# sadit/Jchemo.jl

Hardware: AMD Instinct MI355X
Metric: latent-variables/sec (plskern n=1e6 p=500 q=10 nlv=25) (higher is better)
Workload: dtype f64

## Files before the change

### jchemo.jl_amd/csrc/fit.hip

```cpp
#include <stdlib.h>
#include <time.h>

#include <algorithm>
#include <condition_variable>
#include <mutex>
#include <thread>

#include "jch_internal.h"

__global__ __launch_bounds__(256) void k_fill_const(double *__restrict__ v, int m, double c)
{
    const int j = blockIdx.x * 256 + threadIdx.x;
    if (j < m) v[j] = c;
}

__global__ __launch_bounds__(256) void k_nan_zero_weight_rows(double *__restrict__ T, int64_t n, int nlv, const double *__restrict__ d)
{
    const int64_t i = (int64_t)blockIdx.x * 256 + threadIdx.x;
    if (i < n && d[i] == 0.0)
        for (int a = 0; a < nlv; ++a) T[(size_t)i + (size_t)a * (size_t)n] = __builtin_nan("");
}

__global__ __launch_bounds__(256) void k_widen_bf16(const unsigned short *__restrict__ src, int64_t ld, int64_t n, int64_t cols, double *__restrict__ dst)
{
// ... 151 lines not shown
    const bool host = d.loc == JCH_LOC_HOST;
    const bool inplace = d.inplace != 0;
    ctx->ev_used = 0;
    ctx->prof = jch_profile{};
    jch_coll_reset(ctx);
    ctx->sweep_seq = 0;
    ctx->sweep_alt = jch_knob("JCH_SWEEP_ALT", 0);
    ctx->sweep_fused_reduce = jch_knob("JCH_SWEEP_FUSED_REDUCE", 0) == 1;
    ctx->sweep_resident_mb = jch_knob("JCH_SWEEP_RESIDENT_MB", -1);
    ctx->sweep_tstage = jch_knob("JCH_SWEEP_TSTAGE", -1);
    const bool host_timing = jch_knob_set("JCH_HOST_TIMING");
    auto now_ms = [] { timespec ts; clock_gettime(CLOCK_MONOTONIC, &ts); return ts.tv_sec * 1e3 + ts.tv_nsec * 1e-6; };
    const double tl0 = now_ms();
    double tl_h2d = tl0, tl_enq = tl0, tl_sync = tl0;

    const xcopy_key xkey{io.X, (int64_t)n, (int64_t)io.ldx, p, host ? 1 : 0};
    const bool reuse_x = (d.reserved & JCH_REUSE_XCOPY) && allow_raw && ctx->xcopy_valid && ctx->xcopy == xkey && d.dtype == JCH_F64 &&
                         q + 1 <= 12 && ldr <= 512 && !jch_knob_set("JCH_NO_REUSE_XCOPY");
    if (!reuse_x) ctx->xcopy_valid = false;
    double *Xc = (double *)io.X, *Yc = (double *)io.Y;
    const double *wdev = io.weights;
    int64_t ldxc = io.ldx, ldyc = io.ldy;
    if (host) {
        JCH_TRY(jch_reserve_xstage(ctx, sizeof(double) * (size_t)n * p, reuse_x));
        JCH_TRY(jch_reserve(ctx, ctx->ystage, sizeof(double) * (size_t)n * q));
        Xc = (double *)ctx->xstage.ptr; Yc = (double *)ctx->ystage.ptr; ldxc = n; ldyc = n;
        if (!reuse_x) JCH_TRY(jch_copy2d(ctx, Xc, n, (const double *)io.X, io.ldx, n, p, hipMemcpyHostToDevice));
        JCH_TRY(jch_copy2d(ctx, Yc, n, (const double *)io.Y, io.ldy, n, q, hipMemcpyHostToDevice));
        if (io.weights) {
            JCH_TRY(jch_reserve(ctx, ctx->wstage, sizeof(double) * (size_t)n));
            JCH_HIP(ctx, hipMemcpyAsync(ctx->wstage.ptr, io.weights, sizeof(double) * (size_t)n, hipMemcpyHostToDevice, ctx->stream));
            wdev = (const double *)ctx->wstage.ptr;
        }
    }
    if (host && host_timing) { (void)hipStreamSynchronize(ctx->stream); tl_h2d = now_ms(); }
    const int nlv_cap = (int)std::min<int64_t>(d.nlv, p);
    if (d.dtype == JCH_F64) {
        JCH_TRY(jch_reserve_xr(ctx, sizeof(double) * (size_t)n * ldr, reuse_x));
        JCH_TRY(jch_reserve(ctx, ctx->yr, sizeof(double) * (size_t)n * qpad));
    }
    double *Xr = (double *)ctx->xr.ptr, *Yr = (double *)ctx->yr.ptr;
    double *dn = nullptr;
    if (!host && io.weights_norm) dn = io.weights_norm;
    else { JCH_TRY(jch_reserve(ctx, ctx->dnorm, sizeof(double) * (size_t)n)); dn = (double *)ctx->dnorm.ptr; }
    double *Tdev = nullptr;
    if (!host && io.T) Tdev = io.T;
    else { JCH_TRY(jch_reserve(ctx, ctx->tbuf, sizeof(double) * (size_t)n * nlv_cap)); Tdev = (double *)ctx->tbuf.ptr; }

    t_column_copier tcopy(ctx, (host && d.dtype == JCH_F64 && !(algo == ALGO_WOLD && (d.reserved & JCH_WOLD_REF_ZERO_WEIGHT_NAN))) ? io.T : nullptr, Tdev, n, nlv_cap);
    const size_t small_bytes = 256 * 21 + sizeof(double) * 16 * 2048 + sizeof(double) * (64 + (size_t)p + (size_t)p * qpad + 2 * (size_t)ldr + 3 * (size_t)nlv_cap * p +
                                                         (size_t)nlv_cap * q + 36 * nlv_cap + 1024 + (JCH_ZT_SLICES + 1) * ((size_t)ldr + 8 + qpad) + 2 * (size_t)(p + q) + 8 + 2 * (size_t)ldr + 128 +
                                                         (p <= JCH_SWEEP_MAXP ? jch_lv_split_doubles(p, nlv_cap) + 128 : 0));
    JCH_TRY(jch_reserve(ctx, ctx->small, small_bytes));
// ... 86 lines not shown
        JCH_HIP(ctx, hipStreamSynchronize(ctx->stream));
        n_total = (int64_t)(hdr_h[1] + 0.5);
    }
    const int nlv = (int)std::min<int64_t>(std::min<int64_t>(n_total, p), d.nlv);
    const bool fast = q <= 16 && nlv <= 1024 && p <= JCH_SWEEP_MAXP && jch_lv_fast_lds_bytes(p, q, qpad, ldr, nlv) <= 150 * 1024;
    const bool sib = algo == ALGO_SIMP || algo == ALGO_WOLD;
    const bool sib_fast = sib && jch_sibling_supported(p, q, ldr, nlv);
    const bool all_fast = sib ? (sib_fast && (algo == ALGO_SIMP || fast)) : fast;
    const int max_slices = all_fast ? JCH_ZT_SLICES : 1;
    const bool fuse_inbox = all_fast && ctx->p2p.ready && !ctx->loop &&
                            (size_t)(ldr + 1 + qpad) <= ctx->p2p.cap;
    int nslice = 1;
    const bool ext_scales = io.xscales_in != nullptr;
    const bool raw_mode = (((algo == ALGO_KERN || algo == ALGO_ROSA) && fast) || (algo == ALGO_SIMP && all_fast)) && !ext_scales && !inplace &&
                          q <= 15 && (d.reserved & ~JCH_REUSE_XCOPY) == 0 && p <= JCH_SWEEP_MAXP && allow_raw && !jch_knob_set("JCH_CENTRED_COPY");
    if (raw_mode) {
        s.mshift = mshift_buf;
        double *spread2 = take(p);
        JCH_TRY(jch_launch_pivot(ctx, Xc, ldxc, n, p, s.hdr, s.scl, spread2));
        JCH_TRY(jch_launch_moments(ctx, Yc, ldyc, nullptr, 0, dn, n, q, 0, nullptr, s.scl + p));
        bool from_copy = false;
        if (reuse_x) JCH_TRY(jch_launch_xty_rows(ctx, Xr, ldr, Yc, ldyc, dn, n, p, q, s.scl, Yr, qpad, s.K, s.mom,
                                                 s.mshift, spread2, qual_dev, s.scl, &from_copy));
        if (from_copy) ctx->xcopy_reused++;
        else {
        JCH_TRY(jch_launch_center_xty(ctx, Xc, ldxc, Yc, ldyc, dn, n, p, q, s.scl, s.mom, false, Xr, ldr, Yr, qpad, s.K, false,
                                      s.mom, s.mshift, spread2, qual_dev, s.scl));
        ctx->xcopy = xkey; ctx->xcopy_valid = true;
        }
        if (d.scal) {
            s.rs = take((size_t)ldr + 2);
            JCH_HIP(ctx, hipMemsetAsync(s.rs, 0, sizeof(double) * ((size_t)ldr + 2), ctx->stream));
            JCH_TRY(jch_launch_raw_scales(ctx, Xr, n, p, ldr, dn, s.mshift, Yr, qpad, q, s.zt, s.scl, s.K));
        }
        s.variant = 2;
    } else {
    ctx->xcopy_valid = false;
    JCH_TRY(jch_launch_moments(ctx, Xc, ldxc, Yc, ldyc, dn, n, p, q, nullptr, s.mom));
    if (ext_scales) {
        JCH_TRY(jch_reserve_host(ctx, sizeof(double) * (size_t)(p + q)));
// ... 33 lines not shown
    else if (algo == ALGO_WOLD) JCH_TRY(jch_launch_lv_update(ctx, s, p, q, qpad, ldr, 0 | 0x20000000, nlv, 4, 1, ldz, false, false, nullptr, 0, 0, io.tol, io.maxit));
    else {
        split = (algo == ALGO_KERN || algo == ALGO_ROSA) && fast && jch_knob("JCH_LV_SPLIT", 1) != 0 &&
                jch_lv_solve_lds_bytes(p, q, ldr, nlv) <= 150 * 1024 && (!fuse_inbox || jch_lv_split_p2p_ok(ctx, p));
        if (split) { s.kr = take(16); JCH_TRY(jch_lv_split_begin_fit(ctx, s, take(jch_lv_split_doubles(p, nlv)), p, nlv)); }
        JCH_TRY(jch_launch_lv_update(ctx, s, p, q, qpad, ldr, -1, nlv, kern_like ? 0 : 1, 1, ldz, fast));
    }
    int npend = 0, pend_a0 = 0;
    if (pend_p) JCH_HIP(ctx, hipMemsetAsync(pend_p, 0, sizeof(double) * (size_t)defer_m * jch_nipals_lazy_pitch(ldr), ctx->stream));
    for (int a = 0; a < nlv; ++a) {
        double *tcol = Tdev + (size_t)a * (size_t)n;
        if (kern_like) {
            jch_part_view pv;
            const bool split_fused = split && fuse_inbox;
            JCH_TRY(jch_launch_sweep(ctx, Xr, n, p, ldr, dn, s.rs ? s.rs : s.r, Yr, qpad, 0, tcol, s.zt, ldz, max_slices, &nslice, raw_mode ? s.mshift : nullptr,
                                     split && (ctx->nranks == 1 || split_fused) ? &pv : nullptr));
            tcopy.column_done(a);
            if (ctx->nranks > 1 && max_slices > 1) nslice = JCH_ZT_SLICES;
            if (split) {
                if (!pv.part) {
                    if (!split_fused) JCH_TRY(jch_allreduce_slices(ctx, s.zt, ldr + 1 + (raw_mode ? 1 : 0), nslice, ldz, &nslice));
                    pv.part = s.zt; pv.nb = nslice; pv.ldpart = ldz;
                }
                if (split_fused) ctx->coll_transport = JCH_TRANSPORT_INBOX_FUSED;
                JCH_TRY(jch_launch_lv_split(ctx, s, p, q, ldr, a, nlv, pv.part, pv.nb, pv.ldpart, ldr, raw_mode ? ldr + 1 : -1, raw_mode ? 1 : 0, a + 1 < nlv, split_fused));
                continue;
            }
            if (fuse_inbox && algo != ALGO_SIMP) {
                ctx->coll_transport = JCH_TRANSPORT_INBOX_FUSED;
                JCH_TRY(jch_launch_lv_update(ctx, s, p, q, qpad, ldr, a, nlv, 0, nslice, ldz, fast, true));
            } else {
// ... 231 lines not shown
```

### jchemo.jl_amd/csrc/jch_internal.h

```cpp
#pragma once
#include <hip/hip_runtime.h>
#include <stdint.h>
#include <stdio.h>
#include <string.h>

#include <functional>
#include <string>
#include <vector>

#include "jchemo_hip.h"

#define JCH_MAXQ 64
#define JCH_ZT_SLICES 8
#define JCH_SWEEP_MAXP 2048

struct xcopy_key {
    const void *X; int64_t n, ldx; int p, host;
    bool operator==(const xcopy_key &o) const { return X == o.X && n == o.n && ldx == o.ldx && p == o.p && host == o.host; }
};
struct jch_buf {
    void *ptr = nullptr;
    size_t bytes = 0;
};

struct jch_uid {
    char internal[128];
};
struct jch_rccl {
    void *handle = nullptr;
    int (*GetUniqueId)(void *) = nullptr;
    int (*CommInitRank)(void **, int, jch_uid, int) = nullptr;
    int (*AllReduce)(const void *, void *, size_t, int, int, void *, hipStream_t) = nullptr;
    int (*CommDestroy)(void *) = nullptr;
// ... 150 lines not shown
                              double *Xr, int ldr, double *Yr, int qpad, double *K , bool scal,
                              double *means_out = nullptr ,
                              double *mshift_out = nullptr ,
                              const double *spread2 = nullptr ,
                              double *qual = nullptr ,
                              double *ones_out = nullptr );
int32_t jch_launch_pivot(jch_ctx *ctx, const double *Xc, int64_t ldx, int64_t n, int p, const double *hdr ,
                         double *pivot , double *spread2 );
int32_t jch_launch_export_colmajor(jch_ctx *ctx, const double *Xr, int ldr, const double *Yr, int qpad, int64_t n,
                                   int p, int q, double *Xc, int64_t ldx, double *Yc, int64_t ldy,
                                   const double *sqrt_rowscale = nullptr );
int32_t jch_launch_sweep(jch_ctx *ctx, const double *Xr, int64_t n, int p, int ldr, const double *d, const double *rvec,
                         const double *Yr, int qpad, int q_extra ,
                         double *tcol, double *zt , int ldz, int max_slices,
                         int *nslice_out, const double *mu = nullptr ,
                         jch_part_view *pv = nullptr );
int32_t jch_launch_reduce_rows(jch_ctx *ctx, const double *part, int nb, int ldpart, int m, double *out);
int32_t jch_launch_xty_rows(jch_ctx *ctx, const double *Xr, int ldr, const double *Yc, int64_t ldy, const double *d, int64_t n, int p, int q,
                            const double *mom, double *Yr, int qpad, double *K, double *means_out, double *mshift_out,
                            const double *spread2, double *qual, double *ones_out, bool *done);
int32_t jch_launch_raw_scales(jch_ctx *ctx, const double *Xr, int64_t n, int p, int ldr, const double *d, const double *mshift,
                              const double *Yr, int qpad, int q, double *tmp, double *scl, double *K);
int32_t jch_launch_reduce_part8(jch_ctx *ctx, const double *part, int nb, int ldpart, int m, double *zt, int ldz, int *nslice_out);
int32_t jch_launch_sweep_wide(jch_ctx *ctx, const double *Xr, int64_t n, int ldr, const double *d, const double *rvec,
                              const double *Yr, int qpad, bool nipals, double *tcol, double *zt);
int32_t jch_launch_ytdt(jch_ctx *ctx, const double *Yr, int64_t n, int qpad, const double *d, const double *tcol, double *out );
#define JCH_NIPALS_DEFER_DEFAULT 6
static inline int jch_nipals_lazy_pitch(int ldr) { return 128 * (ldr <= 128 ? 1 : ldr <= 256 ? 2 : ldr <= 512 ? 4 : ldr <= 1024 ? 8 : 16); }
int32_t jch_sweep_tickets(jch_ctx *ctx, int **out);
int jch_nipals_lazy_capacity(int ldr, int q);
int32_t jch_launch_sweep_lazy(jch_ctx *ctx, const double *Xr, int64_t n, int ldr, const double *d, const double *wvec,
                              const double *Yr, int qpad, double *tcol, double *zt, int ldz, int max_slices, int *nslice_out,
                              const double *pend_p, int npend, int npend_max, const double *tpend, int64_t tstride);
int32_t jch_launch_kpass_lazy(jch_ctx *ctx, double *Xr, int64_t n, int p, int ldr, double *Yr, int qpad, int q, const double *d,
                              const double *pend_p, int npend, int npend_max, const double *tpend, int64_t tstride,
// ... 140 lines not shown
```

### jchemo.jl_amd/csrc/prologue.hip

```cpp
#include <stdint.h>
#include <stdlib.h>

#include <algorithm>

#include "jch_internal.h"
#include "rowsum_dev.h"

typedef double v4f64 __attribute__((ext_vector_type(4)));

__global__ __launch_bounds__(256) void k_wsum_part(const double *__restrict__ w, int64_t n, double *__restrict__ part)
{
    __shared__ double sc[4];
    double s = 0.0;
    for (int64_t i = (int64_t)blockIdx.x * 256 + threadIdx.x; i < n; i += (int64_t)gridDim.x * 256) s += w[i];
    s = jch_block_sum<256>(s, sc);
    if (threadIdx.x == 0) part[blockIdx.x] = s;
}

__global__ __launch_bounds__(256) void k_wsum_final(const double *__restrict__ part, int nb, int64_t n, int have_w,
                                                    double *__restrict__ hdr, double *__restrict__ zero0, int nzero0,
                                                    double *__restrict__ zero1, int nzero1)
{
    __shared__ double sc[4];
    for (int i = threadIdx.x; i < nzero0; i += 256) zero0[i] = 0.0;
// ... 394 lines not shown
            }
        }
    }
    double *kp = Kpart + ((size_t)blockIdx.x * kp_rows) * 16;
#pragma unroll
    for (int ct = 0; ct < 8; ++ct)
        if (ct < ntile) {
#pragma unroll
            for (int reg = 0; reg < 4; ++reg) {
                const int j = cg0 + 64 * ct + 16 * wv + (lane >> 4) + 4 * reg;
                if (j < kp_rows) kp[(size_t)j * 16 + (lane & 15)] = acc[ct][reg];
            }
        }
}

__global__ __launch_bounds__(256) void k_reduce_kpart_wide(const double *__restrict__ Kpart, int nbx, int kp_rows, int p, int qpad,
                                                           double *__restrict__ K)
{
    __shared__ double sc[4][64];
    const int el = threadIdx.x & 63, g = threadIdx.x >> 6;
    const int e = blockIdx.x * 64 + el;
    const size_t stride = (size_t)kp_rows * qpad;
    double s0 = 0.0, s1 = 0.0, s2 = 0.0, s3 = 0.0;
    if (e < p * qpad) {
        int b = g;
        for (; b + 12 < nbx; b += 16) {
            s0 += Kpart[(size_t)b * stride + e]; s1 += Kpart[(size_t)(b + 4) * stride + e];
            s2 += Kpart[(size_t)(b + 8) * stride + e]; s3 += Kpart[(size_t)(b + 12) * stride + e];
        }
        for (; b < nbx; b += 4) s0 += Kpart[(size_t)b * stride + e];
// ... 172 lines not shown
    const int nbx = (int)std::max<int64_t>(1, std::min<int64_t>((ngroups + 3) / 4, ctx->cus));
    JCH_TRY(jch_reserve(ctx, ctx->kpart, sizeof(double) * (size_t)nbx * kp_rows * 16));
    double *Kpart = (double *)ctx->kpart.ptr;
    const int nq = q + 1 <= 4 ? 4 : (q + 1 <= 8 ? 8 : 12);
#define JCH_XR(KC, NQ) hipLaunchKernelGGL((k_xty_rows<KC, NQ>), dim3(nbx), dim3(256), sizeof(double) * 4 * KC * 128, ctx->stream, Xr, n, ldr, Yc, ldy, d, q, \
                                          mom + p, ones_col, Yr, Kpart, kp_rows)
#define JCH_XR_NQ(KC) do { if (nq == 4) JCH_XR(KC, 4); else if (nq == 8) JCH_XR(KC, 8); else JCH_XR(KC, 12); } while (0)
    if (kc == 1) JCH_XR_NQ(1); else if (kc == 2) JCH_XR_NQ(2); else if (kc == 3) JCH_XR_NQ(3); else JCH_XR_NQ(4);
#undef JCH_XR_NQ
#undef JCH_XR
    hipLaunchKernelGGL(k_reduce_kpart_wide, dim3((p * 16 + 63) / 64), dim3(256), 0, ctx->stream, Kpart, nbx, kp_rows, p, 16, K);
    JCH_TRY(jch_allreduce_f64(ctx, K, (size_t)p * qpad));
    hipLaunchKernelGGL(k_extract_means, dim3((p + q + 255) / 256), dim3(256), 0, ctx->stream, K, qpad, p, ones_col, mom, means_out, mshift_out, spread2, qual, q, ones_out);
    JCH_HIP(ctx, hipGetLastError());
    *done = true;
    return JCH_OK;
}

int32_t jch_launch_center_xty(jch_ctx *ctx, double *Xc, int64_t ldx, double *Yc, int64_t ldy, const double *d, int64_t n,
                              int p, int q, const double *mom, const double *scl, bool writeback, double *Xr, int ldr,
                              double *Yr, int qpad, double *K, bool scal, double *means_out, double *mshift_out,
                              const double *spread2, double *qual, double *ones_out)
{
    const int ones_col = means_out ? q : -1;
    if (qpad == 16 && ldx % 2 == 0 && ((uintptr_t)Xc) % 16 == 0) {
        const int groups = (ldr + 511) / 512;
        const int kp_rows = groups * 512;
        const int64_t nunits = (n + 31) / 32;
        int nbx = std::max(1, ctx->cus / groups);
        if (nbx > nunits) nbx = (int)nunits;
// ... 97 lines not shown
```

### jchemo.jl_amd/csrc/sweep.hip

```cpp
#include <stdlib.h>

#include <algorithm>

#include "jch_internal.h"

typedef double v2f64 __attribute__((ext_vector_type(2)));

template <int KC, int R, bool NIPALS, bool PF>
__global__ __launch_bounds__(256) void k_sweep(const double *__restrict__ Xr, int64_t n, int ldr,
                                               const double *__restrict__ dw, const double *__restrict__ rvec,
                                               const double *__restrict__ Yr, int qpad, double *__restrict__ tcol,
                                               double *__restrict__ part, int ldpart, const double *__restrict__ mu)
{
    extern __shared__ __attribute__((aligned(16))) double red[];
    const int lane = threadIdx.x & 63, wv = threadIdx.x >> 6, nw = blockDim.x >> 6;
    v2f64 rf[KC], zp[KC];
    bool in[KC];
#pragma unroll
    for (int k = 0; k < KC; ++k) {
        const int col = 2 * lane + 128 * k;
        in[k] = col < ldr;
        rf[k] = in[k] ? *reinterpret_cast<const v2f64 *>(rvec + col) : v2f64{0.0, 0.0};
        zp[k] = v2f64{0.0, 0.0};
    }
// ... 127 lines not shown
        }
        double t = 0.0;
#pragma unroll
        for (int g = 0; g < 16; ++g) t += sg[g];
        zt[(size_t)slice * ldz + c] = t;
    }
    if (slice == 0) {
        const int used = (nb + per - 1) / per;
        for (int e = threadIdx.x; e < (JCH_ZT_SLICES - used) * m; e += blockDim.x) {
            const int sl = used + e / m, c = e - (e / m) * m;
            zt[(size_t)sl * ldz + c] = 0.0;
        }
    }
}

template <int KC, int R, int NBUF, bool NT = true, bool MIX = false, bool TSTAGE = false>
__global__ __launch_bounds__(256) void k_sweep_v2(const double *__restrict__ Xr, int64_t n, int ldr,
                                                  const double *__restrict__ dw, const double *__restrict__ rvec,
                                                  double *__restrict__ tcol, double *__restrict__ part, int ldpart,
                                                  const double *__restrict__ mu, int *__restrict__ tickets,
                                                  double *__restrict__ zt, int ldz, int nslice, int rev = 0, int nres = 0, int tcap = 0)
{
    extern __shared__ __attribute__((aligned(16))) double red[];
    const int lane = threadIdx.x & 63, wv = threadIdx.x >> 6, nw = blockDim.x >> 6;
    v2f64 rf[KC], zp[KC];
    int coff[KC];
#pragma unroll
    for (int k = 0; k < KC; ++k) {
        const int col = 2 * lane + 128 * k;
        coff[k] = col < ldr ? col : ldr - 2;
        zp[k] = v2f64{0.0, 0.0};
    }
    const int64_t ngroups = (n + R - 1) / R;
    const int64_t gstride = (int64_t)gridDim.x * nw;
    v2f64 X[NBUF][R][KC];
    double D[NBUF][R];
    const int64_t gbase = rev ? ngroups - 1 : 0, gsign = rev ? -1 : 1;
    auto fetch = [&](auto nt, v2f64 (&xb)[R][KC], double (&db)[R], int64_t gg) {
        const int64_t r0 = (gbase + gsign * gg) * R;
#pragma unroll
        for (int rr = 0; rr < R; ++rr) {
            const int64_t row = r0 + rr < n ? r0 + rr : n - 1;
            const double *rp = Xr + (size_t)row * (size_t)ldr;
#pragma unroll
            for (int k = 0; k < KC; ++k) {
                if constexpr (decltype(nt)::value) xb[rr][k] = __builtin_nontemporal_load(reinterpret_cast<const v2f64 *>(rp + coff[k]));
                else xb[rr][k] = *reinterpret_cast<const v2f64 *>(rp + coff[k]);
            }
            db[rr] = dw[row];
        }
    };
    double tt = 0.0, st = 0.0, off = 0.0;
    double *tring = red + nw * KC * 128 + 16 + (TSTAGE ? __builtin_amdgcn_readfirstlane(wv) * tcap * R : 0);
    int tfill = 0;
    int64_t tdone = 0;
    auto tflush = [&] {
        const int nf = __builtin_amdgcn_readfirstlane(tfill);
        const int64_t gfirst = (int64_t)blockIdx.x * nw + wv;
        __builtin_amdgcn_fence(__ATOMIC_ACQ_REL, "wavefront");
        for (int s = 0; s < nf; s += 64 / R) {
            const int slot = s + lane / R;
            if (slot < nf) {
                const int64_t row = (gbase + gsign * (gfirst + (tdone + slot) * gstride)) * R + lane % R;
                const double v = tring[s * R + lane];
                if (row < n) tcol[row] = v;
            }
        }
        __builtin_amdgcn_fence(__ATOMIC_ACQ_REL, "wavefront");
        tdone += nf;
        tfill = 0;
    };
    auto coefficients = [&] {
#pragma unroll
        for (int k = 0; k < KC; ++k) rf[k] = 2 * lane + 128 * k < ldr ? *reinterpret_cast<const v2f64 *>(rvec + 2 * lane + 128 * k) : v2f64{0.0, 0.0};
        if (mu) {
            double o = 0.0;
#pragma unroll
            for (int k = 0; k < KC; ++k) {
                const v2f64 m2 = *reinterpret_cast<const v2f64 *>(mu + coff[k]);
                o += m2.x * rf[k].x + m2.y * rf[k].y;
            }
            off = jch_wave_sum(o);
        }
    };
    auto process = [&](v2f64 (&x)[R][KC], double (&dv)[R], int64_t gg) {
        const int64_t row0 = (gbase + gsign * gg) * R;
        double s[R];
#pragma unroll
        for (int rr = 0; rr < R; ++rr) {
            double a = 0.0;
#pragma unroll
            for (int k = 0; k < KC; ++k) a += x[rr][k].x * rf[k].x + x[rr][k].y * rf[k].y;
            s[rr] = a;
        }
        const double h = jch_rowsums<R>(s, lane) - off;
#pragma unroll
        for (int rr = 0; rr < R; ++rr) {
            const double t = jch_readlane(h, jch_rowsum_lane<R>(rr));
            const double dt = row0 + rr < n ? dv[rr] * t : 0.0;
            tt += dt * t;
            st += dt;
// ... 20 lines not shown
        for (int b = 0; b < NBUF - 1; ++b)
            if (g + b * gstride < ngroups) fetch(nt, X[b], D[b], g + b * gstride);
        coefficients();
        while (g < ngroups) {
#pragma unroll
            for (int b = 0; b < NBUF; ++b) {
                if (g < ngroups) {
                    const int64_t ahead = g + (NBUF - 1) * gstride;
                    if (ahead < ngroups) fetch(nt, X[(b + NBUF - 1) % NBUF], D[(b + NBUF - 1) % NBUF], ahead);
                    process(X[b], D[b], g);
                    g += gstride;
                }
            }
        }
    };
    if constexpr (MIX) {
        const unsigned W = gridDim.x * nw, wme = blockIdx.x * nw + __builtin_amdgcn_readfirstlane(wv);
        const unsigned w = rev ? (unsigned)((ngroups - 1) % W + W - wme) % W : wme;
        if (((w + 1u) * (unsigned)nres) / W > (w * (unsigned)nres) / W) stream(std::false_type{});
        else stream(std::true_type{});
    } else {
        stream(std::integral_constant<bool, NT>{});
    }
    if constexpr (TSTAGE) tflush();
    double *zred = red;
    double *tred = red + nw * KC * 128;
#pragma unroll
    for (int k = 0; k < KC; ++k)
        *reinterpret_cast<v2f64 *>(zred + wv * (KC * 128) + 2 * lane + 128 * k) = zp[k];
    if (lane == 0) { tred[wv] = tt; tred[8 + wv] = st; }
    __syncthreads();
    double *prow = part + (size_t)blockIdx.x * ldpart;
    for (int c = threadIdx.x; c < ldr; c += blockDim.x) {
        double a = 0.0;
        for (int w = 0; w < nw; ++w) a += zred[w * (KC * 128) + c];
        jch_publish(prow + c, a, nslice > 0);
    }
    if (threadIdx.x == 0) {
        double a = 0.0, a2 = 0.0;
        for (int w = 0; w < nw; ++w) { a += tred[w]; a2 += tred[8 + w]; }
        jch_publish(prow + ldr, a, nslice > 0);
        if (mu) jch_publish(prow + ldr + 1, a2, nslice > 0);
    }
    jch_slice_sum_by_last_block(part, ldpart, ldr + 1 + (mu ? 1 : 0), tickets, zt, ldz, nslice);
// ... 198 lines not shown
    *nslice_out = nslice;
    JCH_HIP(ctx, hipGetLastError());
    return JCH_OK;
}

int32_t jch_sweep_tickets(jch_ctx *ctx, int **out)
{
    if (!ctx->tickets.ptr) {
        JCH_TRY(jch_reserve(ctx, ctx->tickets, 256));
        JCH_HIP(ctx, hipMemsetAsync(ctx->tickets.ptr, 0, 256, ctx->stream));
    }
    *out = (int *)ctx->tickets.ptr;
    return JCH_OK;
}

template <int KC, int R, int NBUF>
static int32_t launch_sweep_v2_t(jch_ctx *ctx, const double *Xr, int64_t n, int ldr, const double *d, const double *rvec,
                                 double *tcol, double *zt, int ldz, int max_slices, int *nslice_out, int m, const double *mu,
                                 jch_part_view *pv)
{
    const int64_t ngroups = (n + R - 1) / R;
    const size_t lds0 = sizeof(double) * (4 * KC * 128 + 16);
    constexpr bool WIDE = KC == 4 || KC == 8;
    constexpr int TCAP_MAX = WIDE ? (int)((64 * 1024 - sizeof(double) * (4 * KC * 128 + 16)) / (sizeof(double) * 4 * R)) : 0;
    const int tstage = ctx->sweep_tstage;
    const bool staged = WIDE && !ctx->sweep_alt && (tstage > 0 || (tstage < 0 && jch_sweep_tstage_default(KC, n, ctx->cus)));
    static int bpc2[2] = {0, 0};
    static jch_per_device_once once;
    if (!once.done(ctx->device)) {
        int nblk = 0;
        hipError_t e = hipOccupancyMaxActiveBlocksPerMultiprocessor(&nblk, k_sweep_v2<KC, R, NBUF, true>, 256, lds0);
        bpc2[0] = bpc2[1] = (e == hipSuccess && nblk > 0) ? nblk : 1;
        if constexpr (WIDE) {
            e = hipOccupancyMaxActiveBlocksPerMultiprocessor(&nblk, k_sweep_v2<KC, R, NBUF, true, false, true>, 256,
                                                             lds0 + sizeof(double) * 4 * TCAP_MAX * R);
            bpc2[1] = (e == hipSuccess && nblk > 0) ? nblk : 1;
        }
        once.mark(ctx->device);
    }
    const int bpc = bpc2[staged];
    int64_t nb64 = (ngroups + 3) / 4;
    int64_t cap = (int64_t)ctx->cus * bpc;
    if ((KC == 4 || KC == 8) && bpc == 1) cap = std::max<int64_t>(8, (((int64_t)ctx->cus * (n < (int64_t)1280 * ctx->cus ? 14 : 13)) / 16) & ~(int64_t)7);
    if (nb64 > cap) nb64 = cap;
    if (nb64 < 1) nb64 = 1;
    const int nb = (int)nb64;
    const int ldpart = (m + 7) & ~7;
    JCH_TRY(jch_reserve(ctx, ctx->part, sizeof(double) * (size_t)nb * ldpart));
    double *part = (double *)ctx->part.ptr;
    int tcap = 0;
    if (staged) tcap = (int)std::max<int64_t>(1, std::min<int64_t>(std::min(tstage > 0 ? tstage : TCAP_MAX, TCAP_MAX), (ngroups + (int64_t)nb * 4 - 1) / ((int64_t)nb * 4)));
    const size_t lds = lds0 + sizeof(double) * 4 * (size_t)tcap * R;
    int nslice = std::max(1, std::min(JCH_ZT_SLICES, nb / 8));
    const bool fused = ctx->sweep_fused_reduce;
    int *tickets = nullptr;
    if (fused) JCH_TRY(jch_sweep_tickets(ctx, &tickets));
    const bool timed = jch_prof_sample(ctx);
    if (timed) (void)jch_ev(ctx);
    const int alt = ctx->sweep_alt;
    if (alt) {
        const int rev = alt == 2 ? 0 : (int)(ctx->sweep_seq++ & 1u);
        hipLaunchKernelGGL((k_sweep_v2<KC, R, NBUF, false>), dim3(nb), dim3(256), lds, ctx->stream, Xr, n, ldr, d, rvec, tcol, part, ldpart, mu,
                           tickets, zt, ldz, fused ? nslice : 0, rev);
    } else {
    const bool first = ctx->sweep_seq++ == 0u;
    int resident_mb = ctx->sweep_resident_mb;
    if (resident_mb < 0)
        resident_mb = KC == 4 && (double)n * ldr * sizeof(double) >= 7.0 * JCH_INFINITY_CACHE_MIB * 1048576.0 ? JCH_RESIDENT_DEFAULT_MIB : 0;
    int nres = 0;
    if constexpr (KC == 4 || KC == 8)
    if (resident_mb > 0 && bpc == 1) {
        const int64_t W = (int64_t)nb * 4;
        const double wave_bytes = (double)ngroups / (double)W * R * ldr * sizeof(double);
        nres = (int)std::max<int64_t>(1, std::min<int64_t>(W, (int64_t)(std::min(resident_mb, JCH_INFINITY_CACHE_MIB) * 1048576.0 / wave_bytes)));
    }
    if (nres > 0 && tcap > 0)
        hipLaunchKernelGGL((k_sweep_v2<KC, R, NBUF, true, WIDE, WIDE>), dim3(nb), dim3(256), lds, ctx->stream, Xr, n, ldr, d, rvec, tcol, part, ldpart, mu,
                           tickets, zt, ldz, fused ? nslice : 0, first ? 1 : 0, nres, tcap);
    else if (nres > 0)
        hipLaunchKernelGGL((k_sweep_v2<KC, R, NBUF, true, WIDE>), dim3(nb), dim3(256), lds, ctx->stream, Xr, n, ldr, d, rvec, tcol, part, ldpart, mu,
                           tickets, zt, ldz, fused ? nslice : 0, first ? 1 : 0, nres);
    else if (tcap > 0)
        hipLaunchKernelGGL((k_sweep_v2<KC, R, NBUF, true, false, WIDE>), dim3(nb), dim3(256), lds, ctx->stream, Xr, n, ldr, d, rvec, tcol, part, ldpart, mu,
                           tickets, zt, ldz, fused ? nslice : 0, first ? 1 : 0, 0, tcap);
    else
        hipLaunchKernelGGL((k_sweep_v2<KC, R, NBUF, true>), dim3(nb), dim3(256), lds, ctx->stream, Xr, n, ldr, d, rvec, tcol, part, ldpart, mu,
                           tickets, zt, ldz, fused ? nslice : 0, first ? 1 : 0);
    }
    if (timed) (void)jch_ev(ctx);
    if (pv && !fused) {
        pv->part = part; pv->nb = nb; pv->ldpart = ldpart;
        *nslice_out = 1;
        JCH_HIP(ctx, hipGetLastError());
        return JCH_OK;
    }
    if (!fused)
        hipLaunchKernelGGL(k_reduce_part, dim3((m + 63) / 64, JCH_ZT_SLICES), dim3(1024), 0, ctx->stream, part, nb, ldpart, m, nslice, zt, ldz);
    if (nslice > 1) nslice = JCH_ZT_SLICES;
    if (max_slices == 1 && nslice > 1) {
        hipLaunchKernelGGL(k_reduce_slices, dim3((m + 255) / 256), dim3(256), 0, ctx->stream, zt, ldz, m, nslice);
        nslice = 1;
// ... 174 lines not shown
                              const double *pend_p, int npend, int npend_max, const double *tpend, int64_t tstride)
{
    if (npend < 0 || npend > npend_max || npend_max > jch_nipals_lazy_capacity(ldr, 1)) return jch_fail(ctx, JCH_EINVAL, "internal: lazy NIPALS sweep: bad pending count");
#define JCH_SL(KC, R) return launch_sweep_lazy_t<KC, R>(ctx, Xr, n, ldr, d, wvec, Yr, qpad, tcol, zt, ldz, max_slices, nslice_out, pend_p, npend, npend_max, tpend, tstride)
    if (ldr <= 128) JCH_SL(1, 4);
    if (ldr <= 256) JCH_SL(2, 4);
    if (ldr <= 512) JCH_SL(4, 4);
    if (ldr <= 1024) JCH_SL(8, 2);
    if (ldr <= 2048) JCH_SL(16, 2);
#undef JCH_SL
    return jch_fail(ctx, JCH_EINVAL, "internal: lazy NIPALS sweep needs p <= 2048");
}

int32_t jch_launch_sweep(jch_ctx *ctx, const double *Xr, int64_t n, int p, int ldr, const double *d, const double *rvec,
                         const double *Yr, int qpad, int q_extra, double *tcol, double *zt, int ldz, int max_slices,
                         int *nslice_out, const double *mu, jch_part_view *pv)
{
    (void)p;
    const bool nip = q_extra > 0;
    if (pv) *pv = jch_part_view{};
    if (mu && (nip || ldr > JCH_SWEEP_MAXP)) return jch_fail(ctx, JCH_EINVAL, "internal: raw-mode sweep is for plskern-shaped fits with p <= %d", JCH_SWEEP_MAXP);
    const int m = ldr + 1 + (nip ? qpad : (mu ? 1 : 0));
    if (!nip) {
#define JCH_SWEEP_V2_CASE(KC, R, NB) return launch_sweep_v2_t<KC, R, NB>(ctx, Xr, n, ldr, d, rvec, tcol, zt, ldz, max_slices, nslice_out, m, mu, pv)
        if (ldr <= 128) JCH_SWEEP_V2_CASE(1, 8, 2);
        if (ldr <= 256) JCH_SWEEP_V2_CASE(2, 8, 2);
        if (ldr <= 512) {
            if (n < (int64_t)1280 * ctx->cus) JCH_SWEEP_V2_CASE(4, 4, 3);
            JCH_SWEEP_V2_CASE(4, 8, 2);
        }
        if (ldr <= 1024) JCH_SWEEP_V2_CASE(8, 4, 2);
#undef JCH_SWEEP_V2_CASE
    }
#define JCH_SWEEP_CASE(KC, R, PF) return launch_sweep_t<KC, R, PF>(ctx, Xr, n, ldr, d, rvec, Yr, qpad, nip, tcol, zt, ldz, max_slices, nslice_out, m, mu)
    if (ldr <= 128) JCH_SWEEP_CASE(1, 4, false);
// ... 9 lines not shown
```

Baseline: 1547.

## Add grouped 8-row interleaved X copy layout for the p<=512 sweep

Adds a grouped layout for the centred X copy, stored as blocks of 8 rows with columns interleaved in pairs. It comes with a new MFMA-based prologue kernel that writes this layout while computing X'Y, and a GROUPED variant of the v2 sweep kernel that walks it with contiguous vector loads. By default it is used when ldr is in (256,512] and n is large, which covers p=500, n=1e6. The aim is to give every wave a contiguous block per row group and fuse copy with cross-product, but it adds extra LDS, a padded buffer and a new reduction path.

```diff
diff --git a/jchemo.jl_amd/csrc/fit.hip b/jchemo.jl_amd/csrc/fit.hip
--- a/jchemo.jl_amd/csrc/fit.hip
+++ b/jchemo.jl_amd/csrc/fit.hip
@@ -189,7 +189,11 @@
     const double tl0 = now_ms();
     double tl_h2d = tl0, tl_enq = tl0, tl_sync = tl0;
 
-    const xcopy_key xkey{io.X, (int64_t)n, (int64_t)io.ldx, p, host ? 1 : 0};
+    const int grouped_knob = jch_knob("JCH_XCOPY_GROUPED", -1);
+    const bool cols_aligned = host ? n % 2 == 0 : (io.ldx % 2 == 0 && ((uintptr_t)io.X) % 16 == 0);
+    const bool want_grouped = d.dtype == JCH_F64 && !d.scal && !inplace && cols_aligned && q <= 15 && ldr <= 512 && grouped_knob != 0 &&
+                              (grouped_knob == 1 || (ldr > 256 && n >= (int64_t)1280 * ctx->cus));
+    const xcopy_key xkey{io.X, (int64_t)n, (int64_t)io.ldx, p, host ? 1 : 0, want_grouped ? JCH_XCOPY_GROUPED : JCH_XCOPY_ROWMAJOR};
     const bool reuse_x = (d.reserved & JCH_REUSE_XCOPY) && allow_raw && ctx->xcopy_valid && ctx->xcopy == xkey && d.dtype == JCH_F64 &&
                          q + 1 <= 12 && ldr <= 512 && !jch_knob_set("JCH_NO_REUSE_XCOPY");
     if (!reuse_x) ctx->xcopy_valid = false;
@@ -211,7 +215,7 @@
     if (host && host_timing) { (void)hipStreamSynchronize(ctx->stream); tl_h2d = now_ms(); }
     const int nlv_cap = (int)std::min<int64_t>(d.nlv, p);
     if (d.dtype == JCH_F64) {
-        JCH_TRY(jch_reserve_xr(ctx, sizeof(double) * (size_t)n * ldr, reuse_x));
+        JCH_TRY(jch_reserve_xr(ctx, sizeof(double) * (size_t)(want_grouped ? (n + 7) / 8 * 8 : n) * ldr, reuse_x));
         JCH_TRY(jch_reserve(ctx, ctx->yr, sizeof(double) * (size_t)n * qpad));
     }
     double *Xr = (double *)ctx->xr.ptr, *Yr = (double *)ctx->yr.ptr;
@@ -328,16 +332,26 @@
     const bool ext_scales = io.xscales_in != nullptr;
     const bool raw_mode = (((algo == ALGO_KERN || algo == ALGO_ROSA) && fast) || (algo == ALGO_SIMP && all_fast)) && !ext_scales && !inplace &&
                           q <= 15 && (d.reserved & ~JCH_REUSE_XCOPY) == 0 && p <= JCH_SWEEP_MAXP && allow_raw && !jch_knob_set("JCH_CENTRED_COPY");
+    const bool grouped = raw_mode && want_grouped;
     if (raw_mode) {
         s.mshift = mshift_buf;
         double *spread2 = take(p);
         JCH_TRY(jch_launch_pivot(ctx, Xc, ldxc, n, p, s.hdr, s.scl, spread2));
         JCH_TRY(jch_launch_moments(ctx, Yc, ldyc, nullptr, 0, dn, n, q, 0, nullptr, s.scl + p));
         bool from_copy = false;
+        if (reuse_x && grouped) {
+            JCH_TRY(jch_launch_center_xty_grouped(ctx, Xr, 0, true, Yc, ldyc, dn, n, p, q, s.scl, nullptr, ldr, Yr, s.K, s.mom,
+                                                  s.mshift, spread2, qual_dev, s.scl));
+            from_copy = true;
+        } else
         if (reuse_x) JCH_TRY(jch_launch_xty_rows(ctx, Xr, ldr, Yc, ldyc, dn, n, p, q, s.scl, Yr, qpad, s.K, s.mom,
                                                  s.mshift, spread2, qual_dev, s.scl, &from_copy));
         if (from_copy) ctx->xcopy_reused++;
         else {
+        if (grouped)
+            JCH_TRY(jch_launch_center_xty_grouped(ctx, Xc, ldxc, false, Yc, ldyc, dn, n, p, q, s.scl, Xr, ldr, Yr, s.K, s.mom,
+                                                  s.mshift, spread2, qual_dev, s.scl));
+        else
         JCH_TRY(jch_launch_center_xty(ctx, Xc, ldxc, Yc, ldyc, dn, n, p, q, s.scl, s.mom, false, Xr, ldr, Yr, qpad, s.K, false,
                                       s.mom, s.mshift, spread2, qual_dev, s.scl));
         ctx->xcopy = xkey; ctx->xcopy_valid = true;
@@ -401,7 +415,7 @@
             jch_part_view pv;
             const bool split_fused = split && fuse_inbox;
             JCH_TRY(jch_launch_sweep(ctx, Xr, n, p, ldr, dn, s.rs ? s.rs : s.r, Yr, qpad, 0, tcol, s.zt, ldz, max_slices, &nslice, raw_mode ? s.mshift : nullptr,
-                                     split && (ctx->nranks == 1 || split_fused) ? &pv : nullptr));
+                                     split && (ctx->nranks == 1 || split_fused) ? &pv : nullptr, grouped));
             tcopy.column_done(a);
             if (ctx->nranks > 1 && max_slices > 1) nslice = JCH_ZT_SLICES;
             if (split) {
diff --git a/jchemo.jl_amd/csrc/jch_internal.h b/jchemo.jl_amd/csrc/jch_internal.h
--- a/jchemo.jl_amd/csrc/jch_internal.h
+++ b/jchemo.jl_amd/csrc/jch_internal.h
@@ -14,9 +14,10 @@
 #define JCH_ZT_SLICES 8
 #define JCH_SWEEP_MAXP 2048
 
+enum { JCH_XCOPY_ROWMAJOR = 0, JCH_XCOPY_GROUPED = 1 };
 struct xcopy_key {
-    const void *X; int64_t n, ldx; int p, host;
-    bool operator==(const xcopy_key &o) const { return X == o.X && n == o.n && ldx == o.ldx && p == o.p && host == o.host; }
+    const void *X; int64_t n, ldx; int p, host, layout;
+    bool operator==(const xcopy_key &o) const { return X == o.X && n == o.n && ldx == o.ldx && p == o.p && host == o.host && layout == o.layout; }
 };
 struct jch_buf {
     void *ptr = nullptr;
@@ -197,11 +198,15 @@
                          const double *Yr, int qpad, int q_extra ,
                          double *tcol, double *zt , int ldz, int max_slices,
                          int *nslice_out, const double *mu = nullptr ,
-                         jch_part_view *pv = nullptr );
+                         jch_part_view *pv = nullptr ,
+                         bool grouped = false );
 int32_t jch_launch_reduce_rows(jch_ctx *ctx, const double *part, int nb, int ldpart, int m, double *out);
 int32_t jch_launch_xty_rows(jch_ctx *ctx, const double *Xr, int ldr, const double *Yc, int64_t ldy, const double *d, int64_t n, int p, int q,
                             const double *mom, double *Yr, int qpad, double *K, double *means_out, double *mshift_out,
                             const double *spread2, double *qual, double *ones_out, bool *done);
+int32_t jch_launch_center_xty_grouped(jch_ctx *ctx, const double *Xsrc, int64_t ldx, bool from_copy, const double *Yc, int64_t ldy, const double *d,
+                                      int64_t n, int p, int q, const double *mom, double *Xg, int ldr, double *Yr, double *K, double *means_out,
+                                      double *mshift_out, const double *spread2, double *qual, double *ones_out);
 int32_t jch_launch_raw_scales(jch_ctx *ctx, const double *Xr, int64_t n, int p, int ldr, const double *d, const double *mshift,
                               const double *Yr, int qpad, int q, double *tmp, double *scl, double *K);
 int32_t jch_launch_reduce_part8(jch_ctx *ctx, const double *part, int nb, int ldpart, int m, double *zt, int ldz, int *nslice_out);
diff --git a/jchemo.jl_amd/csrc/prologue.hip b/jchemo.jl_amd/csrc/prologue.hip
--- a/jchemo.jl_amd/csrc/prologue.hip
+++ b/jchemo.jl_amd/csrc/prologue.hip
@@ -432,6 +432,111 @@
         }
 }
 
+template <bool FROMCOPY>
+__global__ __launch_bounds__(256) void k_center_xty_grouped(const double *__restrict__ Xsrc, int64_t ldx, const double *__restrict__ Yc, int64_t ldy,
+                                                            const double *__restrict__ d, int64_t n, int p, int q, const double *__restrict__ mom,
+                                                            double *__restrict__ Xg, int ldr, double *__restrict__ Yr, double *__restrict__ Kpart,
+                                                            int kp_rows, int ones_col)
+{
+    constexpr int NP = 4;
+    typedef double v4f64p __attribute__((ext_vector_type(4)));
+    const int lane = threadIdx.x & 63, wv = threadIdx.x >> 6;
+    const int cl = lane & 15, rp = lane >> 4;
+    const int cw0 = 128 * wv;
+    const int64_t last_even = (n - 1) & ~(int64_t)1;
+    const int64_t ngrp = (n + 7) / 8;
+    const size_t gpitch = (size_t)8 * (size_t)ldr;
+    double cm[8];
+    size_t cbase[8];
+#pragma unroll
+    for (int ct = 0; ct < 8; ++ct) {
+        const int j = cw0 + 16 * ct + cl;
+        cm[ct] = (!FROMCOPY && j < p) ? mom[j] : 0.0;
+        cbase[ct] = FROMCOPY ? (size_t)min(j, ldr - 1) * 8 + 2 * rp : (size_t)min(j, p - 1) * (size_t)ldx;
+    }
+    const double ym = cl < q ? mom[p + cl] : 0.0;
+    const int yc_ = min(cl, q - 1);
+    v4f64p acc[8];
+#pragma unroll
+    for (int t = 0; t < 8; ++t) acc[t] = v4f64p{0.0, 0.0, 0.0, 0.0};
+    v2f64p Rg[NP][8];
+    double yraw[16], draw[16], breg[16];
+    auto fetch = [&](v2f64p (&rb)[8], int64_t t0, size_t cb) {
+#pragma unroll
+        for (int g = 0; g < 8; ++g) {
+            if constexpr (FROMCOPY) {
+                const int64_t grp = min(t0 / 8 + g, ngrp - 1);
+                rb[g] = __builtin_nontemporal_load(reinterpret_cast<const v2f64p *>(Xsrc + (size_t)grp * gpitch + cb));
+            } else {
+                const int64_t i = min(t0 + 8 * g + 2 * rp, last_even);
+                rb[g] = __builtin_nontemporal_load(reinterpret_cast<const v2f64p *>(Xsrc + cb + (size_t)i));
+            }
+        }
+    };
+    auto yload = [&](int64_t t0) {
+#pragma unroll
+        for (int e = 0; e < 16; ++e) {
+            const int64_t row = min(t0 + 8 * (e >> 1) + 2 * rp + (e & 1), n - 1);
+            draw[e] = d[row];
+            yraw[e] = Yc[(size_t)row + (size_t)yc_ * (size_t)ldy];
+        }
+    };
+    auto bbuild = [&](int64_t t0) {
+#pragma unroll
+        for (int e = 0; e < 16; ++e) {
+            const int64_t row = t0 + 8 * (e >> 1) + 2 * rp + (e & 1);
+            const bool ok = row < n;
+            const double yv = (ok && cl < q) ? yraw[e] - ym : 0.0;
+            const double dv = ok ? draw[e] : 0.0;
+            if (ok && wv == 0) Yr[(size_t)row * 16 + cl] = yv;
+            breg[e] = cl == ones_col ? dv : dv * yv;
+        }
+    };
+    int64_t i0 = (int64_t)blockIdx.x * 64;
+    const int64_t istep = (int64_t)gridDim.x * 64;
+    if (cw0 < ldr && i0 < n) {
+        yload(i0);
+#pragma unroll
+        for (int b = 0; b < NP - 1; ++b) fetch(Rg[b], i0, cbase[b]);
+        bbuild(i0);
+        yload(min(i0 + istep, n - 1));
+        for (; i0 < n; i0 += istep) {
+#pragma unroll
+            for (int ct = 0; ct < 8; ++ct) {
+                constexpr int AH = NP - 1;
+                fetch(Rg[(ct + AH) % NP], ct + AH < 8 ? i0 : i0 + istep, cbase[(ct + AH) % 8]);
+                const int j = cw0 + 16 * ct + cl;
+                const bool jlive = j < p;
+#pragma unroll
+                for (int g = 0; g < 8; ++g) {
+                    const int64_t i = i0 + 8 * g + 2 * rp;
+                    v2f64p v = Rg[ct % NP][g];
+                    if constexpr (!FROMCOPY) { v.x -= cm[ct]; v.y -= cm[ct]; }
+                    if (!(jlive && i < n)) v.x = 0.0;
+                    if (!(jlive && i + 1 < n)) v.y = 0.0;
+                    if constexpr (!FROMCOPY) {
+                        if (j < ldr && i0 + 8 * g < n)
+                            __builtin_nontemporal_store(v, reinterpret_cast<v2f64p *>(Xg + (size_t)(i0 / 8 + g) * gpitch + (size_t)j * 8 + 2 * rp));
+                    }
+                    acc[ct] = __builtin_amdgcn_mfma_f64_16x16x4f64(v.x, breg[2 * g], acc[ct], 0, 0, 0);
+                    acc[ct] = __builtin_amdgcn_mfma_f64_16x16x4f64(v.y, breg[2 * g + 1], acc[ct], 0, 0, 0);
+                }
+            }
+            bbuild(i0 + istep);
+            yload(min(i0 + 2 * istep, n - 1));
+        }
+    }
+    double *kp = Kpart + ((size_t)blockIdx.x * kp_rows) * 16;
+#pragma unroll
+    for (int ct = 0; ct < 8; ++ct) {
+#pragma unroll
+        for (int reg = 0; reg < 4; ++reg) {
+            const int j = cw0 + 16 * ct + rp + 4 * reg;
+            if (j < kp_rows) kp[(size_t)j * 16 + cl] = acc[ct][reg];
+        }
+    }
+}
+
 __global__ __launch_bounds__(256) void k_reduce_kpart_wide(const double *__restrict__ Kpart, int nbx, int kp_rows, int p, int qpad,
                                                            double *__restrict__ K)
 {
@@ -634,6 +739,27 @@
     hipLaunchKernelGGL(k_extract_means, dim3((p + q + 255) / 256), dim3(256), 0, ctx->stream, K, qpad, p, ones_col, mom, means_out, mshift_out, spread2, qual, q, ones_out);
     JCH_HIP(ctx, hipGetLastError());
     *done = true;
+    return JCH_OK;
+}
+
+int32_t jch_launch_center_xty_grouped(jch_ctx *ctx, const double *Xsrc, int64_t ldx, bool from_copy, const double *Yc, int64_t ldy, const double *d,
+                                      int64_t n, int p, int q, const double *mom, double *Xg, int ldr, double *Yr, double *K, double *means_out,
+                                      double *mshift_out, const double *spread2, double *qual, double *ones_out)
+{
+    if (q > 15 || ldr > 512 || ldr < 2 || !means_out || (!from_copy && (ldx % 2 != 0 || ((uintptr_t)Xsrc) % 16 != 0)))
+        return jch_fail(ctx, JCH_EINVAL, "internal: grouped prologue outside its envelope");
+    const int ones_col = q, kp_rows = 512;
+    const int nbx = (int)std::max<int64_t>(1, std::min<int64_t>((n + 63) / 64, ctx->cus));
+    JCH_TRY(jch_reserve(ctx, ctx->kpart, sizeof(double) * (size_t)nbx * kp_rows * 16));
+    double *Kpart = (double *)ctx->kpart.ptr;
+    if (from_copy)
+        hipLaunchKernelGGL(k_center_xty_grouped<true>, dim3(nbx), dim3(256), 0, ctx->stream, Xsrc, ldx, Yc, ldy, d, n, p, q, mom, Xg, ldr, Yr, Kpart, kp_rows, ones_col);
+    else
+        hipLaunchKernelGGL(k_center_xty_grouped<false>, dim3(nbx), dim3(256), 0, ctx->stream, Xsrc, ldx, Yc, ldy, d, n, p, q, mom, Xg, ldr, Yr, Kpart, kp_rows, ones_col);
+    hipLaunchKernelGGL(k_reduce_kpart_wide, dim3((p * 16 + 63) / 64), dim3(256), 0, ctx->stream, Kpart, nbx, kp_rows, p, 16, K);
+    JCH_TRY(jch_allreduce_f64(ctx, K, (size_t)p * 16));
+    hipLaunchKernelGGL(k_extract_means, dim3((p + q + 255) / 256), dim3(256), 0, ctx->stream, K, 16, p, ones_col, mom, means_out, mshift_out, spread2, qual, q, ones_out);
+    JCH_HIP(ctx, hipGetLastError());
     return JCH_OK;
 }
 
diff --git a/jchemo.jl_amd/csrc/sweep.hip b/jchemo.jl_amd/csrc/sweep.hip
--- a/jchemo.jl_amd/csrc/sweep.hip
+++ b/jchemo.jl_amd/csrc/sweep.hip
@@ -165,7 +165,7 @@
     }
 }
 
-template <int KC, int R, int NBUF, bool NT = true, bool MIX = false, bool TSTAGE = false>
+template <int KC, int R, int NBUF, bool NT = true, bool MIX = false, bool TSTAGE = false, bool GROUPED = false>
 __global__ __launch_bounds__(256) void k_sweep_v2(const double *__restrict__ Xr, int64_t n, int ldr,
                                                   const double *__restrict__ dw, const double *__restrict__ rvec,
                                                   double *__restrict__ tcol, double *__restrict__ part, int ldpart,
@@ -173,8 +173,21 @@
                                                   double *__restrict__ zt, int ldz, int nslice, int rev = 0, int nres = 0, int tcap = 0)
 {
     extern __shared__ __attribute__((aligned(16))) double red[];
+    static_assert(!GROUPED || (KC == 4 && R == 8), "the grouped walk is the 500-column R = 8 sweep's");
+    constexpr int NM = R * KC;
     const int lane = threadIdx.x & 63, wv = threadIdx.x >> 6, nw = blockDim.x >> 6;
+    const int ga = lane & 3, gq = lane >> 2;
     v2f64 rf[KC], zp[KC];
+    double zg[GROUPED ? NM : 1];
+    double *rl = red + nw * KC * 128 + 16;
+    const int glast = 8 * (ldr - 1) + 2 * ga;
+    const int gmf = ldr >> 4;
+    const int gedge = 16 * gmf + gq < ldr ? 2 * lane + 128 * gmf : glast;
+    const int wvu = __builtin_amdgcn_readfirstlane(wv);
+    if constexpr (GROUPED) {
+#pragma unroll
+        for (int m = 0; m < NM; ++m) zg[m] = 0.0;
+    }
     int coff[KC];
 #pragma unroll
     for (int k = 0; k < KC; ++k) {
@@ -187,8 +200,20 @@
     v2f64 X[NBUF][R][KC];
     double D[NBUF][R];
     const int64_t gbase = rev ? ngroups - 1 : 0, gsign = rev ? -1 : 1;
-    auto fetch = [&](auto nt, v2f64 (&xb)[R][KC], double (&db)[R], int64_t gg) {
+    auto fetch = [&](auto nt, v2f64 (&xb)[R][KC], double (&db)[R], int64_t gg) __attribute__((always_inline)) {
         const int64_t r0 = (gbase + gsign * gg) * R;
+        if constexpr (GROUPED) {
+            const double *gp = Xr + (size_t)r0 * (size_t)ldr;
+#pragma unroll
+            for (int m = 0; m < NM; ++m) {
+                const int o = m < gmf ? 2 * lane + 128 * m : (m == gmf ? gedge : glast);
+                if constexpr (decltype(nt)::value) xb[m / KC][m % KC] = __builtin_nontemporal_load(reinterpret_cast<const v2f64 *>(gp + o));
+                else xb[m / KC][m % KC] = *reinterpret_cast<const v2f64 *>(gp + o);
+            }
+#pragma unroll
+            for (int u = 0; u < 2; ++u) db[u] = dw[r0 + 2 * ga + u < n ? r0 + 2 * ga + u : n - 1];
+            return;
+        }
 #pragma unroll
         for (int rr = 0; rr < R; ++rr) {
             const int64_t row = r0 + rr < n ? r0 + rr : n - 1;
@@ -202,7 +227,7 @@
         }
     };
     double tt = 0.0, st = 0.0, off = 0.0;
-    double *tring = red + nw * KC * 128 + 16 + (TSTAGE ? __builtin_amdgcn_readfirstlane(wv) * tcap * R : 0);
+    double *tring = red + nw * KC * 128 + 16 + (GROUPED ? 512 : 0) + (TSTAGE ? __builtin_amdgcn_readfirstlane(wv) * tcap * R : 0);
     int tfill = 0;
     int64_t tdone = 0;
     auto tflush = [&] {
@@ -221,7 +246,29 @@
         tdone += nf;
         tfill = 0;
     };
+    double rpre[2];
+    if constexpr (GROUPED) {
+#pragma unroll
+        for (int u = 0; u < 2; ++u) rpre[u] = rvec[min((int)threadIdx.x + 256 * u, ldr - 1)];
+    }
     auto coefficients = [&] {
+        if constexpr (GROUPED) {
+            double mv[8];
+            if (mu) {
+#pragma unroll
+                for (int k = 0; k < 8; ++k) mv[k] = mu[min(lane + 64 * k, ldr - 1)];
+            }
+#pragma unroll
+            for (int u = 0; u < 2; ++u) rl[threadIdx.x + 256 * u] = (int)threadIdx.x + 256 * u < ldr ? rpre[u] : 0.0;
+            __syncthreads();
+            if (mu) {
+                double o = 0.0;
+#pragma unroll
+                for (int k = 0; k < 8; ++k) o += mv[k] * rl[lane + 64 * k];
+                off = jch_wave_sum(o);
+            }
+            return;
+        }
 #pragma unroll
         for (int k = 0; k < KC; ++k) rf[k] = 2 * lane + 128 * k < ldr ? *reinterpret_cast<const v2f64 *>(rvec + 2 * lane + 128 * k) : v2f64{0.0, 0.0};
         if (mu) {
@@ -236,6 +283,39 @@
     };
     auto process = [&](v2f64 (&x)[R][KC], double (&dv)[R], int64_t gg) {
         const int64_t row0 = (gbase + gsign * gg) * R;
+        if constexpr (GROUPED) {
+            double s0 = 0.0, s1 = 0.0;
+#pragma unroll
+            for (int m = 0; m < NM; ++m) {
+                const double rm = rl[16 * m + gq];
+                s0 += x[m / KC][m % KC].x * rm;
+                s1 += x[m / KC][m % KC].y * rm;
+            }
+            jch_fold32(s0, s1);
+            { double c = s0; jch_fold16(s0, c); }
+            s0 += jch_dpp<0x128>(s0);
+            s0 += jch_dpp<0x124>(s0);
+            const double h = s0 - off;
+            const v2u32 lo = __builtin_amdgcn_permlane32_swap((unsigned)__double2loint(h), (unsigned)__double2loint(h), false, false);
+            const v2u32 hi = __builtin_amdgcn_permlane32_swap((unsigned)__double2hiint(h), (unsigned)__double2hiint(h), false, false);
+            const double t0 = __hiloint2double((int)hi.x, (int)lo.x), t1 = __hiloint2double((int)hi.y, (int)lo.y);
+            const double dt0 = row0 + 2 * ga < n ? dv[0] * t0 : 0.0, dt1 = row0 + 2 * ga + 1 < n ? dv[1] * t1 : 0.0;
+            tt += dt0 * t0; tt += dt1 * t1;
+            st += dt0; st += dt1;
+#pragma unroll
+            for (int m = 0; m < NM; ++m) {
+                zg[m] += dt0 * x[m / KC][m % KC].x;
+                zg[m] += dt1 * x[m / KC][m % KC].y;
+            }
+            const double tl = __shfl(h, ((lane >> 1) & 3) + 32 * (lane & 1), 64);
+            if constexpr (TSTAGE) {
+                if (lane < R) tring[tfill * R + lane] = tl;
+                if (__builtin_amdgcn_readfirstlane(++tfill) == tcap) tflush();
+            } else {
+                if (lane < R && row0 + lane < n) tcol[row0 + lane] = tl;
+            }
+            return;
+        }
         double s[R];
 #pragma unroll
         for (int rr = 0; rr < R; ++rr) {
@@ -286,20 +366,62 @@
             }
         }
     };
+    auto stream_g = [&](bool resident) {
+        auto fetch_g = [&](v2f64 (&xb)[R][KC], double (&db)[R], int64_t gg) __attribute__((always_inline)) {
+            if constexpr (MIX) {
+                if (resident) fetch(std::false_type{}, xb, db, gg);
+                else fetch(std::true_type{}, xb, db, gg);
+            } else {
+                fetch(std::integral_constant<bool, NT>{}, xb, db, gg);
+            }
+        };
+        int64_t g = (int64_t)blockIdx.x * nw + wvu;
+#pragma unroll
+        for (int b = 0; b < NBUF - 1; ++b)
+            if (g + b * gstride < ngroups) fetch_g(X[b], D[b], g + b * gstride);
+        coefficients();
+        while (g < ngroups) {
+#pragma unroll
+            for (int b = 0; b < NBUF; ++b) {
+                if (g < ngroups) {
+                    const int64_t ahead = g + (NBUF - 1) * gstride;
+                    if (ahead < ngroups) fetch_g(X[(b + NBUF - 1) % NBUF], D[(b + NBUF - 1) % NBUF], ahead);
+                    process(X[b], D[b], g);
+                    g += gstride;
+                }
+            }
+        }
+    };
     if constexpr (MIX) {
         const unsigned W = gridDim.x * nw, wme = blockIdx.x * nw + __builtin_amdgcn_readfirstlane(wv);
         const unsigned w = rev ? (unsigned)((ngroups - 1) % W + W - wme) % W : wme;
-        if (((w + 1u) * (unsigned)nres) / W > (w * (unsigned)nres) / W) stream(std::false_type{});
+        const bool resident = ((w + 1u) * (unsigned)nres) / W > (w * (unsigned)nres) / W;
+        if constexpr (GROUPED) stream_g(resident);
+        else if (resident) stream(std::false_type{});
         else stream(std::true_type{});
+    } else if constexpr (GROUPED) {
+        stream_g(false);
     } else {
         stream(std::integral_constant<bool, NT>{});
     }
     if constexpr (TSTAGE) tflush();
     double *zred = red;
     double *tred = red + nw * KC * 128;
+    if constexpr (GROUPED) {
+#pragma unroll
+        for (int m = 0; m < NM; ++m) {
+            double v = zg[m];
+            v += jch_dpp<0xB1>(v);
+            v += jch_dpp<0x4E>(v);
+            if (ga == 0) zred[wv * (KC * 128) + 16 * m + gq] = v;
+        }
+        tt = ((jch_readlane(tt, 0) + jch_readlane(tt, 1)) + jch_readlane(tt, 2)) + jch_readlane(tt, 3);
+        st = ((jch_readlane(st, 0) + jch_readlane(st, 1)) + jch_readlane(st, 2)) + jch_readlane(st, 3);
+    } else {
 #pragma unroll
     for (int k = 0; k < KC; ++k)
         *reinterpret_cast<v2f64 *>(zred + wv * (KC * 128) + 2 * lane + 128 * k) = zp[k];
+    }
     if (lane == 0) { tred[wv] = tt; tred[8 + wv] = st; }
     __syncthreads();
     double *prow = part + (size_t)blockIdx.x * ldpart;
@@ -528,25 +650,25 @@
     return JCH_OK;
 }
 
-template <int KC, int R, int NBUF>
+template <int KC, int R, int NBUF, bool G = false>
 static int32_t launch_sweep_v2_t(jch_ctx *ctx, const double *Xr, int64_t n, int ldr, const double *d, const double *rvec,
                                  double *tcol, double *zt, int ldz, int max_slices, int *nslice_out, int m, const double *mu,
                                  jch_part_view *pv)
 {
     const int64_t ngroups = (n + R - 1) / R;
-    const size_t lds0 = sizeof(double) * (4 * KC * 128 + 16);
+    const size_t lds0 = sizeof(double) * (4 * KC * 128 + 16 + (G ? 512 : 0));
     constexpr bool WIDE = KC == 4 || KC == 8;
-    constexpr int TCAP_MAX = WIDE ? (int)((64 * 1024 - sizeof(double) * (4 * KC * 128 + 16)) / (sizeof(double) * 4 * R)) : 0;
+    constexpr int TCAP_MAX = WIDE ? (int)((64 * 1024 - sizeof(double) * (4 * KC * 128 + 16 + (G ? 512 : 0))) / (sizeof(double) * 4 * R)) : 0;
     const int tstage = ctx->sweep_tstage;
     const bool staged = WIDE && !ctx->sweep_alt && (tstage > 0 || (tstage < 0 && jch_sweep_tstage_default(KC, n, ctx->cus)));
     static int bpc2[2] = {0, 0};
     static jch_per_device_once once;
     if (!once.done(ctx->device)) {
         int nblk = 0;
-        hipError_t e = hipOccupancyMaxActiveBlocksPerMultiprocessor(&nblk, k_sweep_v2<KC, R, NBUF, true>, 256, lds0);
+        hipError_t e = hipOccupancyMaxActiveBlocksPerMultiprocessor(&nblk, k_sweep_v2<KC, R, NBUF, true, false, false, G>, 256, lds0);
         bpc2[0] = bpc2[1] = (e == hipSuccess && nblk > 0) ? nblk : 1;
         if constexpr (WIDE) {
-            e = hipOccupancyMaxActiveBlocksPerMultiprocessor(&nblk, k_sweep_v2<KC, R, NBUF, true, false, true>, 256,
+            e = hipOccupancyMaxActiveBlocksPerMultiprocessor(&nblk, k_sweep_v2<KC, R, NBUF, true, false, true, G>, 256,
                                                              lds0 + sizeof(double) * 4 * TCAP_MAX * R);
             bpc2[1] = (e == hipSuccess && nblk > 0) ? nblk : 1;
         }
@@ -574,7 +696,7 @@
     const int alt = ctx->sweep_alt;
     if (alt) {
         const int rev = alt == 2 ? 0 : (int)(ctx->sweep_seq++ & 1u);
-        hipLaunchKernelGGL((k_sweep_v2<KC, R, NBUF, false>), dim3(nb), dim3(256), lds, ctx->stream, Xr, n, ldr, d, rvec, tcol, part, ldpart, mu,
+        hipLaunchKernelGGL((k_sweep_v2<KC, R, NBUF, false, false, false, G>), dim3(nb), dim3(256), lds, ctx->stream, Xr, n, ldr, d, rvec, tcol, part, ldpart, mu,
                            tickets, zt, ldz, fused ? nslice : 0, rev);
     } else {
     const bool first = ctx->sweep_seq++ == 0u;
@@ -589,16 +711,16 @@
         nres = (int)std::max<int64_t>(1, std::min<int64_t>(W, (int64_t)(std::min(resident_mb, JCH_INFINITY_CACHE_MIB) * 1048576.0 / wave_bytes)));
     }
     if (nres > 0 && tcap > 0)
-        hipLaunchKernelGGL((k_sweep_v2<KC, R, NBUF, true, WIDE, WIDE>), dim3(nb), dim3(256), lds, ctx->stream, Xr, n, ldr, d, rvec, tcol, part, ldpart, mu,
+        hipLaunchKernelGGL((k_sweep_v2<KC, R, NBUF, true, WIDE, WIDE, G>), dim3(nb), dim3(256), lds, ctx->stream, Xr, n, ldr, d, rvec, tcol, part, ldpart, mu,
                            tickets, zt, ldz, fused ? nslice : 0, first ? 1 : 0, nres, tcap);
     else if (nres > 0)
-        hipLaunchKernelGGL((k_sweep_v2<KC, R, NBUF, true, WIDE>), dim3(nb), dim3(256), lds, ctx->stream, Xr, n, ldr, d, rvec, tcol, part, ldpart, mu,
+        hipLaunchKernelGGL((k_sweep_v2<KC, R, NBUF, true, WIDE, false, G>), dim3(nb), dim3(256), lds, ctx->stream, Xr, n, ldr, d, rvec, tcol, part, ldpart, mu,
                            tickets, zt, ldz, fused ? nslice : 0, first ? 1 : 0, nres);
     else if (tcap > 0)
-        hipLaunchKernelGGL((k_sweep_v2<KC, R, NBUF, true, false, WIDE>), dim3(nb), dim3(256), lds, ctx->stream, Xr, n, ldr, d, rvec, tcol, part, ldpart, mu,
+        hipLaunchKernelGGL((k_sweep_v2<KC, R, NBUF, true, false, WIDE, G>), dim3(nb), dim3(256), lds, ctx->stream, Xr, n, ldr, d, rvec, tcol, part, ldpart, mu,
                            tickets, zt, ldz, fused ? nslice : 0, first ? 1 : 0, 0, tcap);
     else
-        hipLaunchKernelGGL((k_sweep_v2<KC, R, NBUF, true>), dim3(nb), dim3(256), lds, ctx->stream, Xr, n, ldr, d, rvec, tcol, part, ldpart, mu,
+        hipLaunchKernelGGL((k_sweep_v2<KC, R, NBUF, true, false, false, G>), dim3(nb), dim3(256), lds, ctx->stream, Xr, n, ldr, d, rvec, tcol, part, ldpart, mu,
                            tickets, zt, ldz, fused ? nslice : 0, first ? 1 : 0);
     }
     if (timed) (void)jch_ev(ctx);
@@ -803,11 +925,15 @@
 
 int32_t jch_launch_sweep(jch_ctx *ctx, const double *Xr, int64_t n, int p, int ldr, const double *d, const double *rvec,
                          const double *Yr, int qpad, int q_extra, double *tcol, double *zt, int ldz, int max_slices,
-                         int *nslice_out, const double *mu, jch_part_view *pv)
+                         int *nslice_out, const double *mu, jch_part_view *pv, bool grouped)
 {
     (void)p;
     const bool nip = q_extra > 0;
     if (pv) *pv = jch_part_view{};
+    if (grouped) {
+        if (nip || !mu || ldr > 512 || ldr < 2) return jch_fail(ctx, JCH_EINVAL, "internal: the grouped copy is for raw-mode plskern-shaped fits with p <= 512");
+        return launch_sweep_v2_t<4, 8, 2, true>(ctx, Xr, n, ldr, d, rvec, tcol, zt, ldz, max_slices, nslice_out, ldr + 2, mu, pv);
+    }
     if (mu && (nip || ldr > JCH_SWEEP_MAXP)) return jch_fail(ctx, JCH_EINVAL, "internal: raw-mode sweep is for plskern-shaped fits with p <= %d", JCH_SWEEP_MAXP);
     const int m = ldr + 1 + (nip ? qpad : (mu ? 1 : 0));
     if (!nip) {
```

After: 1379. 0.892x the previous value.
